# CodyRichter/MLMicroserviceTemplate

Measured on AMD Instinct MI355X. Metric: requests/sec (whole node) + p50 latency, ResNet-50 bs=32, higher is better.
Workload: dtype bf16; 1 GPU; model=resnet50-v1.5, global_batch=32, per_gpu_batch=32, image_size=224, parallelism=dp1, backend=fused, concurrent_slots=True, cu_partitions=2, hipgraph=True, inflight=4, numa_bound=True, partition_mode=intra, prestage=False, ranks_consistent=True, dist_backend=none, dist_world=1

## Files before the change

mlmicroservicetemplate_amd/ops/csrc/conv_chain.hip:

```cpp
#include "common.h"
#include "fastdiv.h"

namespace {

#define LDS3 __attribute__((address_space(3)))

MLS_DEV void glds16(rsrc_t r, char* lds, int voff, int soff) {
  __builtin_amdgcn_raw_ptr_buffer_load_lds(r, (LDS3 void*)lds, 16, voff, soff, 0, 0);
}

typedef unsigned int u32x4v __attribute__((__vector_size__(16)));

MLS_DEV uint32_t lds_off(const void* p);
MLS_DEV u32x4v lds_ld16_issue(uint32_t off);
template <typename T>
MLS_DEV void lds_landed(T& v);

#define CONST4 __attribute__((address_space(4)))

MLS_DEV f32x4 bias4(const float* b, int nt0, int fq) {
  if (!b) return f32x4{0.f, 0.f, 0.f, 0.f};
  const CONST4 f32x4* bp = (const CONST4 f32x4*)(b + nt0);
  const f32x4 b0 = bp[0], b1 = bp[1], b2 = bp[2], b3 = bp[3];
  return fq == 0 ? b0 : fq == 1 ? b1 : fq == 2 ? b2 : b3;
}

struct ChainArgs {
  const bf16* a1;
  const bf16* a2;
  const bf16* w3;
  const float* b3;
  const bf16* res;
  bf16* y;
  const bf16* w1;
  const float* b1;
  bf16* t1;
  int M, Ka, Kb, N1, N2;
  int Ho, Wo, H2, W2, stride2;
  FastDiv fd_howo, fd_wo;
  uint32_t a1_bytes, a2_bytes, w3_bytes, res_bytes, y_bytes, w1_bytes, t1_bytes;
  const bf16* t1in;
  const bf16* w2;
  const float* b2;
  uint32_t t1in_bytes, w2_bytes;
};

template <int CPR>
MLS_DEV int row_swz(int r) {
  if constexpr (CPR == 8) return r & 7;
  else return (r & 1) | ((r >> 1) & 2);
}

template <int BM, int KS, int N1, int N2, int CW, int OCC, bool SW, bool C2 = false>
__global__ __launch_bounds__(512, OCC) void conv_chain_kernel(const ChainArgs a) {
  constexpr int NW = 8, NT = 512, WM = 4, WN = 2;
  constexpr int WTM = BM / WM, TM = WTM / 16;
  constexpr int TN = CW / WN / 16;
  constexpr int TN2 = N2 / WN / 16;
  constexpr int CPR = CW / 8;
  constexpr int RPP = 64 / CPR;
  constexpr int A1_BYTES = BM * KS * 128;
  constexpr int W3_BYTES = CW * KS * 128;
  constexpr int W1_BYTES = N2 * CW * 2;
  constexpr int R_BYTES = BM * CW * 2;
  constexpr int STAGE = W3_BYTES + W1_BYTES + R_BYTES;
  constexpr int EPI_BYTES = BM * N2 * 2;
  constexpr int RING = A1_BYTES + 2 * STAGE;
  constexpr int LDS_BYTES = RING > EPI_BYTES ? RING : EPI_BYTES;
  constexpr int A1_PW = BM / 8 * KS / NW;
  constexpr int A1_S0 = C2 ? 1 : 0;
  constexpr int A1_PWL = BM / 8 * (KS - A1_S0) / NW;
  constexpr int W3_PW = CW / 8 * KS / NW;
  constexpr int W1_PW = N2 / RPP / NW;
  constexpr int R_PW = BM / RPP / NW;
  constexpr int Y_ST = BM * CPR / NT;
  constexpr int T_ST = BM * N2 / 8 / NT;
  constexpr int NJ = N1 / CW;
  static_assert(TM >= 1 && TN >= 1 && TN2 >= 1 && (CW == 64 || CW == 32), "tile");
  static_assert(A1_PW * NW * 8 == BM * KS && W3_PW * NW * 8 == CW * KS, "A1 / W3 DMA split");
  static_assert(W1_PW * NW * RPP == N2 && R_PW * NW * RPP == BM, "W1 / residual DMA split");
  static_assert(Y_ST * NT == BM * CPR && T_ST * NT == BM * N2 / 8, "epilogue split");
  static_assert(LDS_BYTES <= 160 * 1024, "LDS");
  __shared__ __attribute__((aligned(16))) char smem[LDS_BYTES];

  const int tid = threadIdx.x, lane = tid & 63;
  const int wid = __builtin_amdgcn_readfirstlane(tid >> 6);
  const int wm = wid / WN, wn = wid % WN;
  const int fr = lane & 15, fq = lane >> 4;
  const int m0 = xcd_remap(blockIdx.x, gridDim.x) * BM;
  const int K1 = a.Ka + a.Kb, KSA = a.Ka / 64;
  const bool has_res = a.res != nullptr;

  float b3v[SW ? 1 : NJ][TN], b1v[TN2];
  if constexpr (!SW) {
#pragma unroll
    for (int j = 0; j < NJ; ++j)
#pragma unroll
      for (int jn = 0; jn < TN; ++jn) b3v[j][jn] = a.b3 ? a.b3[j * CW + wn * (CW / 2) + jn * 16 + fr] : 0.f;
#pragma unroll
    for (int jn = 0; jn < TN2; ++jn) b1v[jn] = a.b1 ? a.b1[wn * (N2 / 2) + jn * 16 + fr] : 0.f;
  }

  const int r8 = lane >> 3, lc = (lane & 7) ^ r8;
  const int rq = lane / CPR, lq = (lane % CPR) ^ row_swz<CPR>(rq);

  const rsrc_t a1r = make_rsrc(a.a1, a.a1_bytes);
  const rsrc_t a2r = make_rsrc(a.a2, a.a2_bytes);
  const rsrc_t w3r = make_rsrc(a.w3, a.w3_bytes);
  const rsrc_t w1r = make_rsrc(a.w1, a.w1_bytes);
  const rsrc_t rr = make_rsrc(a.res, a.res_bytes);
  const rsrc_t yr = make_rsrc(a.y, a.y_bytes);
  const rsrc_t tr = make_rsrc(a.t1, a.t1_bytes);

  char* const sA1 = smem;
  auto stage_base = [&](int buf) { return smem + A1_BYTES + buf * STAGE; };

#pragma unroll
  for (int i = 0; i < A1_PWL; ++i) {
    const int q = A1_S0 * (BM / 8) + wid * A1_PWL + i;
    const int s = q / (BM / 8), rb = q - s * (BM / 8);
    const int m = m0 + rb * 8 + r8;
    char* dst = sA1 + q * 1024;
    if (s < KSA) {
      glds16(a1r, dst, m < a.M ? (m * a.Ka + s * 64 + lc * 8) * 2 : OOB, 0);
    } else {
      int off = OOB;
      if (m < a.M) {
        const int b = fastdiv(m, a.fd_howo), rem = m - b * (a.Ho * a.Wo);
        const int oh = fastdiv(rem, a.fd_wo), ow = rem - oh * a.Wo;
        off = (((b * a.H2 + oh * a.stride2) * a.W2 + ow * a.stride2) * a.Kb + (s - KSA) * 64 + lc * 8) * 2;
      }
      glds16(a2r, dst, off, 0);
    }
  }

  auto issue = [&](int j, int buf) {
    char* sW3 = stage_base(buf);
    char* sW1 = sW3 + W3_BYTES;
    char* sR = sW1 + W1_BYTES;
#pragma unroll
    for (int i = 0; i < W3_PW; ++i) {
      const int q = wid * W3_PW + i;
      const int s = q / (CW / 8), rb = q - s * (CW / 8);
      glds16(w3r, sW3 + q * 1024, ((j * CW + rb * 8 + r8) * K1 + s * 64 + lc * 8) * 2, 0);
    }
#pragma unroll
    for (int i = 0; i < W1_PW; ++i) {
      const int q = wid * W1_PW + i;
      glds16(w1r, sW1 + q * 1024, ((q * RPP + rq) * N1 + j * CW + lq * 8) * 2, 0);
    }
    if (has_res) {
#pragma unroll
      for (int i = 0; i < R_PW; ++i) {
        const int q = wid * R_PW + i;
        const int m = m0 + q * RPP + rq;
        glds16(rr, sR + q * 1024, m < a.M ? (m * N1 + j * CW + lq * 8) * 2 : OOB, 0);
      }
    }
  };

  if constexpr (C2) {
    constexpr int TAPS = 9, TSLOTS = 4, TAHEAD = 3, SROWS = 256, TNP = 64 / WN / 16;
    static_assert(BM == 128 && STAGE >= SROWS * 128 && STAGE >= TSLOTS * 8192, "strip / tap ring alias one stage each");
    char* const sS = stage_base(0);
    char* const sT = stage_base(1);
    const rsrc_t t1r = make_rsrc(a.t1in, a.t1in_bytes);
    const rsrc_t w2r = make_rsrc(a.w2, a.w2_bytes);
    const int halo = a.Wo + 1;
#pragma unroll
    for (int i = 0; i < SROWS / 8 / NW; ++i) {
      const int q = wid * (SROWS / 8 / NW) + i;
      const int sr = q * 8 + r8, p = m0 - halo + sr;
      glds16(t1r, sS + q * 1024, (p >= 0 && p < a.M && sr < BM + 2 * halo) ? (p * 64 + lc * 8) * 2 : OOB, 0);
    }
    auto issue_tap = [&](int t) {
      glds16(w2r, sT + (t % TSLOTS) * 8192 + wid * 1024, (((wid * 8 + r8) * TAPS + t) * 64 + lc * 8) * 2, 0);
    };
#pragma unroll
    for (int t = 0; t < TAHEAD; ++t) issue_tap(t);

    int okm[TM];
#pragma unroll
    for (int i = 0; i < TM; ++i) {
      const int m = m0 + wm * WTM + i * 16 + fr;
      okm[i] = 0;
      if (m < a.M) {
        const int b = fastdiv(m, a.fd_howo), rem = m - b * (a.Ho * a.Wo);
        const int oh = fastdiv(rem, a.fd_wo), ow = rem - oh * a.Wo;
#pragma unroll
        for (int t = 0; t < TAPS; ++t)
          if ((unsigned)(oh + t / 3 - 1) < (unsigned)a.Ho && (unsigned)(ow + t % 3 - 1) < (unsigned)a.Wo)
            okm[i] |= 1 << t;
      }
    }

    f32x4 accp[TM][TNP];
#pragma unroll
    for (int i = 0; i < TM; ++i)
#pragma unroll
      for (int jn = 0; jn < TNP; ++jn) accp[i][jn] = f32x4{0.f, 0.f, 0.f, 0.f};
#pragma unroll
    for (int t = 0; t < TAPS; ++t) {
      if (t + 2 < TAPS) asm volatile("s_waitcnt vmcnt(2)" ::: "memory");
      else if (t + 1 < TAPS) asm volatile("s_waitcnt vmcnt(1)" ::: "memory");
      else asm volatile("s_waitcnt vmcnt(0)" ::: "memory");
      asm volatile("s_waitcnt lgkmcnt(0)" ::: "memory");
      __builtin_amdgcn_s_barrier();
      if (t + TAHEAD < TAPS) issue_tap(t + TAHEAD);
      const int shift = halo + (t / 3 - 1) * a.Wo + (t % 3 - 1);
      const uint32_t oS = lds_off(sS), oT = lds_off(sT + (t % TSLOTS) * 8192);
      u32x4v av[2][TM], bv[2][TNP];
#pragma unroll
      for (int kk = 0; kk < 2; ++kk) {
        const int ch = fq + 4 * kk;
#pragma unroll
        for (int i = 0; i < TM; ++i) {
          const int r = wm * WTM + i * 16 + fr + shift;
          av[kk][i] = lds_ld16_issue(oS + (r * 8 + (ch ^ (r & 7))) * 16);
        }
#pragma unroll
        for (int jn = 0; jn < TNP; ++jn) {
          const int n = wn * 32 + jn * 16 + fr;
          bv[kk][jn] = lds_ld16_issue(oT + (n * 8 + (ch ^ (n & 7))) * 16);
        }
      }
#pragma unroll
      for (int kk = 0; kk < 2; ++kk) {
#pragma unroll
        for (int i = 0; i < TM; ++i) lds_landed(av[kk][i]);
#pragma unroll
        for (int jn = 0; jn < TNP; ++jn) lds_landed(bv[kk][jn]);
      }
#pragma unroll
      for (int kk = 0; kk < 2; ++kk) {
        bf16x8 af[TM], bfv[TNP];
#pragma unroll
        for (int i = 0; i < TM; ++i) {
          u32x4v v = av[kk][i];
          if (!((okm[i] >> t) & 1)) v = u32x4v{0u, 0u, 0u, 0u};
          af[i] = __builtin_bit_cast(bf16x8, v);
        }
#pragma unroll
        for (int jn = 0; jn < TNP; ++jn) bfv[jn] = __builtin_bit_cast(bf16x8, bv[kk][jn]);
#pragma unroll
        for (int i = 0; i < TM; ++i)
#pragma unroll
          for (int jn = 0; jn < TNP; ++jn)
            accp[i][jn] = __builtin_amdgcn_mfma_f32_16x16x32_bf16(bfv[jn], af[i], accp[i][jn], 0, 0, 0);
      }
    }
#pragma unroll
    for (int jn = 0; jn < TNP; ++jn) {
      const int nt0 = wn * 32 + jn * 16, col = nt0 + fq * 4;
      const f32x4 bb = bias4(a.b2, nt0, fq);
#pragma unroll
      for (int i = 0; i < TM; ++i) {
        const int row = wm * WTM + i * 16 + fr;
        bf16x4 q;
#pragma unroll
        for (int r = 0; r < 4; ++r) {
          const float e = accp[i][jn][r];
          q[r] = (bf16)fmaxf(e + bb[r], 0.f);
        }
        *reinterpret_cast<uint2*>(sA1 + row * 128 + (((col >> 3) ^ (row & 7)) << 4) + (col & 7) * 2) =
            __builtin_bit_cast(uint2, q);
      }
    }
    asm volatile("s_waitcnt lgkmcnt(0)" ::: "memory");
    __builtin_amdgcn_s_barrier();
  }
  issue(0, 0);

  f32x4 acc2[TM][TN2];
#pragma unroll
  for (int i = 0; i < TM; ++i)
#pragma unroll
    for (int jn = 0; jn < TN2; ++jn) acc2[i][jn] = f32x4{0.f, 0.f, 0.f, 0.f};

#pragma unroll
  for (int j = 0; j < NJ; ++j) {
    if (j == 0) {
      asm volatile("s_waitcnt vmcnt(0)" ::: "memory");
      if constexpr (!SW) {
#pragma unroll
        for (int jj = 0; jj < NJ; ++jj)
#pragma unroll
          for (int jn = 0; jn < TN; ++jn) asm volatile("" ::"v"(b3v[jj][jn]));
#pragma unroll
        for (int jn = 0; jn < TN2; ++jn) asm volatile("" ::"v"(b1v[jn]));
      }
    } else {
      asm volatile("s_waitcnt vmcnt(%0)" ::"n"(Y_ST) : "memory");
    }
    asm volatile("s_waitcnt lgkmcnt(0)" ::: "memory");
    __builtin_amdgcn_s_barrier();
    if (j + 1 < NJ) issue(j + 1, (j + 1) & 1);
    char* sW3 = stage_base(j & 1);
    char* sW1 = sW3 + W3_BYTES;
    char* sR = sW1 + W1_BYTES;

    f32x4 acc1[TM][TN];
#pragma unroll
    for (int i = 0; i < TM; ++i)
#pragma unroll
      for (int jn = 0; jn < TN; ++jn) acc1[i][jn] = f32x4{0.f, 0.f, 0.f, 0.f};
    const uint4* A1s = reinterpret_cast<const uint4*>(sA1);
    const uint4* W3s = reinterpret_cast<const uint4*>(sW3);
#pragma unroll
    for (int kk = 0; kk < 2 * KS; ++kk) {
      const int s = kk >> 1, ch = fq + 4 * (kk & 1);
      bf16x8 af[TM], bfv[TN];
#pragma unroll
      for (int i = 0; i < TM; ++i) {
        const int r = wm * WTM + i * 16 + fr;
        af[i] = __builtin_bit_cast(bf16x8, A1s[s * BM * 8 + r * 8 + (ch ^ (r & 7))]);
      }
#pragma unroll
      for (int jn = 0; jn < TN; ++jn) {
        const int n = wn * (CW / 2) + jn * 16 + fr;
        bfv[jn] = __builtin_bit_cast(bf16x8, W3s[s * CW * 8 + n * 8 + (ch ^ (n & 7))]);
      }
#pragma unroll
      for (int i = 0; i < TM; ++i)
#pragma unroll
        for (int jn = 0; jn < TN; ++jn)
          acc1[i][jn] = SW ? __builtin_amdgcn_mfma_f32_16x16x32_bf16(bfv[jn], af[i], acc1[i][jn], 0, 0, 0)
                                       : __builtin_amdgcn_mfma_f32_16x16x32_bf16(af[i], bfv[jn], acc1[i][jn], 0, 0, 0);
    }

    if constexpr (SW) {
#pragma unroll
      for (int jn = 0; jn < TN; ++jn) {
        const int nt0 = wn * (CW / 2) + jn * 16, col = nt0 + fq * 4;
        const f32x4 bb = bias4(a.b3, j * CW + nt0, fq);
#pragma unroll
        for (int i = 0; i < TM; ++i) {
          const int row = wm * WTM + i * 16 + fr;
          uint2* p = reinterpret_cast<uint2*>(sR + row * (CW * 2) + (((col >> 3) ^ row_swz<CPR>(row)) << 4) +
                                              (col & 7) * 2);
          float rs[4] = {0.f, 0.f, 0.f, 0.f};
          if (has_res) {
            const bf16x4 rv = __builtin_bit_cast(bf16x4, *p);
#pragma unroll
            for (int r = 0; r < 4; ++r) rs[r] = (float)rv[r];
          }
          bf16x4 q;
#pragma unroll
          for (int r = 0; r < 4; ++r) {
            const float e = acc1[i][jn][r];
            q[r] = (bf16)fmaxf(e + bb[r] + rs[r], 0.f);
          }
          *p = __builtin_bit_cast(uint2, q);
        }
      }
    } else
#pragma unroll
    for (int jn = 0; jn < TN; ++jn) {
      const int col = wn * (CW / 2) + jn * 16 + fr;
      const float bb = b3v[j][jn];
#pragma unroll
      for (int i = 0; i < TM; ++i)
#pragma unroll
        for (int r = 0; r < 4; ++r) {
          const int row = wm * WTM + i * 16 + fq * 4 + r;
          bf16* p = reinterpret_cast<bf16*>(sR + row * (CW * 2) + (((col >> 3) ^ row_swz<CPR>(row)) << 4) +
                                            (col & 7) * 2);
          const float e = acc1[i][jn][r];
          float v = e + bb;
          if (has_res) v += (float)*p;
          *p = (bf16)fmaxf(v, 0.f);
        }
    }
    asm volatile("s_waitcnt lgkmcnt(0)" ::: "memory");
    __builtin_amdgcn_s_barrier();

#pragma unroll
    for (int it = 0; it < Y_ST; ++it) {
      const int q = tid + it * NT;
      const int row = q / CPR, c = q % CPR;
      const uint4 v = *reinterpret_cast<const uint4*>(sR + row * (CW * 2) + ((c ^ row_swz<CPR>(row)) << 4));
      const int m = m0 + row;
      __builtin_amdgcn_raw_buffer_store_b128(__builtin_bit_cast(u32x4v, v), yr,
                                             m < a.M ? (m * N1 + j * CW + c * 8) * 2 : OOB, 0, 0);
    }

    const uint4* Ys = reinterpret_cast<const uint4*>(sR);
    const uint4* W1s = reinterpret_cast<const uint4*>(sW1);
#pragma unroll
    for (int kk = 0; kk < CW / 32; ++kk) {
      const int ch = fq + 4 * kk;
      bf16x8 af[TM], bfv[TN2];
#pragma unroll
      for (int i = 0; i < TM; ++i) {
        const int r = wm * WTM + i * 16 + fr;
        af[i] = __builtin_bit_cast(bf16x8, Ys[r * CPR + (ch ^ row_swz<CPR>(r))]);
      }
#pragma unroll
      for (int jn = 0; jn < TN2; ++jn) {
        const int n = wn * (N2 / 2) + jn * 16 + fr;
        bfv[jn] = __builtin_bit_cast(bf16x8, W1s[n * CPR + (ch ^ row_swz<CPR>(n))]);
      }
#pragma unroll
      for (int i = 0; i < TM; ++i)
#pragma unroll
        for (int jn = 0; jn < TN2; ++jn)
          acc2[i][jn] = SW ? __builtin_amdgcn_mfma_f32_16x16x32_bf16(bfv[jn], af[i], acc2[i][jn], 0, 0, 0)
                                       : __builtin_amdgcn_mfma_f32_16x16x32_bf16(af[i], bfv[jn], acc2[i][jn], 0, 0, 0);
    }
  }

  asm volatile("s_waitcnt lgkmcnt(0)" ::: "memory");
  __builtin_amdgcn_s_barrier();
  constexpr int TPR = N2 / 8;
  bf16* to = reinterpret_cast<bf16*>(smem);
  if constexpr (SW) {
#pragma unroll
    for (int jn = 0; jn < TN2; ++jn) {
      const int nt0 = wn * (N2 / 2) + jn * 16, col = nt0 + fq * 4;
      const f32x4 bb = bias4(a.b1, nt0, fq);
#pragma unroll
      for (int i = 0; i < TM; ++i) {
        const int row = wm * WTM + i * 16 + fr;
        bf16x4 q;
#pragma unroll
        for (int r = 0; r < 4; ++r) {
          const float e = acc2[i][jn][r];
          q[r] = (bf16)fmaxf(e + bb[r], 0.f);
        }
        *reinterpret_cast<uint2*>(to + row * N2 + ((((col >> 3) ^ (row & 7))) << 3) + (col & 7)) =
            __builtin_bit_cast(uint2, q);
      }
    }
  } else
#pragma unroll
  for (int jn = 0; jn < TN2; ++jn) {
    const int col = wn * (N2 / 2) + jn * 16 + fr;
    const float bb = b1v[jn];
#pragma unroll
    for (int i = 0; i < TM; ++i)
#pragma unroll
      for (int r = 0; r < 4; ++r) {
        const int row = wm * WTM + i * 16 + fq * 4 + r;
        const float e = acc2[i][jn][r];
        to[row * N2 + ((((col >> 3) ^ (row & 7))) << 3) + (col & 7)] = (bf16)fmaxf(e + bb, 0.f);
      }
  }
  asm volatile("s_waitcnt lgkmcnt(0)" ::: "memory");
  __builtin_amdgcn_s_barrier();
#pragma unroll
  for (int it = 0; it < T_ST; ++it) {
    const int q = tid + it * NT;
    const int row = q / TPR, c = q - (q / TPR) * TPR;
    const uint4 v = *reinterpret_cast<const uint4*>(to + row * N2 + ((c ^ (row & 7)) << 3));
    const int m = m0 + row;
    __builtin_amdgcn_raw_buffer_store_b128(__builtin_bit_cast(u32x4v, v), tr, m < a.M ? (m * a.N2 + c * 8) * 2 : OOB,
                                           0, 0);
  }
}

MLS_DEV void vm_wait(int n) {
#define MLS_VMW(k) \
  case k: asm volatile("s_waitcnt vmcnt(" #k ")" ::: "memory"); break;
  switch (n) {
    MLS_VMW(1) MLS_VMW(2) MLS_VMW(3) MLS_VMW(4) MLS_VMW(5) MLS_VMW(6) MLS_VMW(7) MLS_VMW(8) MLS_VMW(9) MLS_VMW(10)
    MLS_VMW(11) MLS_VMW(12) MLS_VMW(13) MLS_VMW(14) MLS_VMW(15) MLS_VMW(16) MLS_VMW(17) MLS_VMW(18) MLS_VMW(19)
    MLS_VMW(20)
    default: asm volatile("s_waitcnt vmcnt(0)" ::: "memory");
  }
#undef MLS_VMW
}

MLS_DEV uint32_t lds_off(const void* p) { return (uint32_t)(uintptr_t)(LDS3 const char*)p; }
MLS_DEV uint2 lds_ld8_issue(uint32_t off) {
  uint2 v;
  asm volatile("ds_read_b64 %0, %1" : "=v"(v) : "v"(off) : "memory");
  return v;
}
MLS_DEV uint32_t lds_ld2_issue(uint32_t off) {
  uint32_t v;
  asm volatile("ds_read_u16 %0, %1" : "=v"(v) : "v"(off) : "memory");
  return v;
}
template <typename T>
MLS_DEV void lds_landed(T& v) { asm volatile("s_waitcnt lgkmcnt(0)" : "+v"(v)::"memory"); }
MLS_DEV u32x4v lds_ld16_issue(uint32_t off) {
  u32x4v v;
  asm volatile("ds_read_b128 %0, %1" : "=v"(v) : "v"(off) : "memory");
  return v;
}
MLS_DEV uint4 lds_ld16(uint32_t off) {
  uint4 v;
  asm volatile("ds_read_b128 %0, %1\n\ts_waitcnt lgkmcnt(0)" : "=v"(v) : "v"(off) : "memory");
  return v;
}
MLS_DEV void lds_st8(uint32_t off, uint2 v) { asm volatile("ds_write_b64 %0, %1" ::"v"(off), "v"(v) : "memory"); }
MLS_DEV void lds_st2(uint32_t off, bf16 h) {
  const uint32_t v = __builtin_bit_cast(unsigned short, h);
  asm volatile("ds_write_b16 %0, %1" ::"v"(off), "v"(v) : "memory");
}

template <int BM, int KS, int N1, int N2, int CW, int S, int OCC, bool SW, bool PERS>
__global__ __launch_bounds__(512, OCC) void conv_chain_ring_kernel(const ChainArgs a, const int ntiles) {
  constexpr int NW = 8, NT = 512, WM = 4, WN = 2;
  constexpr int WTM = BM / WM, TM = WTM / 16;
  constexpr int TN = CW / WN / 16;
  constexpr int TN2 = N2 / WN / 16;
  constexpr int CPR = CW / 8;
  constexpr int RPP = 64 / CPR;
  constexpr int NJ = N1 / CW;
  constexpr int A1_BYTES = BM * KS * 128;
  constexpr int W3_BYTES = CW * KS * 128;
  constexpr int W1_BYTES = N2 * CW * 2;
  constexpr int R_BYTES = BM * CW * 2;
  constexpr int EPI_BYTES = BM * N2 * 2;
  constexpr int STAGE = PERS ? R_BYTES : W3_BYTES + W1_BYTES + R_BYTES;
  constexpr int OFF_W3 = (PERS ? 2 : 1) * A1_BYTES;
  constexpr int OFF_W1 = OFF_W3 + (PERS ? NJ * W3_BYTES : 0);
  constexpr int OFF_EPI = OFF_W1 + (PERS ? NJ * W1_BYTES : 0);
  constexpr int OFF_RING = OFF_EPI + (PERS ? EPI_BYTES : 0);
  constexpr int RING_END = OFF_RING + S * STAGE;
  constexpr int LDS_BYTES = RING_END > EPI_BYTES ? RING_END : EPI_BYTES;
  constexpr int A1_P = BM / 8 * KS, W3_P = CW / 8 * KS, W1_P = N2 / RPP, R_P = BM / RPP;
  constexpr int Y_ST = BM * CPR / NT;
  constexpr int T_ST = BM * N2 / 8 / NT;
  static_assert(TM >= 1 && TN >= 1 && TN2 >= 1 && (CW == 64 || CW == 32), "tile");
  static_assert(S >= 2 && S - 1 <= NJ && (!PERS || NJ % S == 0), "ring depth");
  static_assert(Y_ST * NT == BM * CPR && T_ST * NT == BM * N2 / 8, "epilogue split");
  static_assert(LDS_BYTES <= 160 * 1024, "LDS");
  __shared__ __attribute__((aligned(16))) char smem[LDS_BYTES];

  const int tid = threadIdx.x, lane = tid & 63;
  const int wid = __builtin_amdgcn_readfirstlane(tid >> 6);
  const int wm = wid / WN, wn = wid % WN;
  const int fr = lane & 15, fq = lane >> 4;
  const int G = gridDim.x;
  int tile = chain_first_tile(blockIdx.x, G);
  if (tile >= ntiles) return;
  int m0 = tile * BM;
  const int K1 = a.Ka + a.Kb, KSA = a.Ka / 64;
  const bool has_res = a.res != nullptr;

  float b3v[SW ? 1 : NJ][TN], b1v[TN2];
  if constexpr (!SW) {
#pragma unroll
    for (int j = 0; j < NJ; ++j)
#pragma unroll
      for (int jn = 0; jn < TN; ++jn) b3v[j][jn] = a.b3 ? a.b3[j * CW + wn * (CW / 2) + jn * 16 + fr] : 0.f;
#pragma unroll
    for (int jn = 0; jn < TN2; ++jn) b1v[jn] = a.b1 ? a.b1[wn * (N2 / 2) + jn * 16 + fr] : 0.f;
  }

  const int r8 = lane >> 3, lc = (lane & 7) ^ r8;
  const int rq = lane / CPR, lq = (lane % CPR) ^ row_swz<CPR>(rq);

  const rsrc_t a1r = make_rsrc(a.a1, a.a1_bytes);
  const rsrc_t a2r = make_rsrc(a.a2, a.a2_bytes);
  const rsrc_t w3r = make_rsrc(a.w3, a.w3_bytes);
  const rsrc_t w1r = make_rsrc(a.w1, a.w1_bytes);
  const rsrc_t rr = make_rsrc(a.res, a.res_bytes);
  const rsrc_t yr = make_rsrc(a.y, a.y_bytes);
  const rsrc_t tr = make_rsrc(a.t1, a.t1_bytes);

  auto pieces = [&](int P) { return P / NW + (wid < P % NW ? 1 : 0); };
  const int n_a1 = pieces(A1_P);
  const int n_st = (PERS ? 0 : pieces(W3_P) + pieces(W1_P)) + (has_res ? pieces(R_P) : 0);

  auto issue_a1 = [&](int mt, char* dstA) {
#pragma unroll
    for (int i = 0; i < (A1_P + NW - 1) / NW; ++i) {
      const int q = i * NW + wid;
      if (A1_P % NW != 0 && q >= A1_P) break;
      const int s = q / (BM / 8), rb = q - s * (BM / 8);
      const int m = mt + rb * 8 + r8;
      char* dst = dstA + q * 1024;
      if (s < KSA) {
        glds16(a1r, dst, m < a.M ? (m * a.Ka + s * 64 + lc * 8) * 2 : OOB, 0);
      } else {
        int off = OOB;
        if (m < a.M) {
          const int b = fastdiv(m, a.fd_howo), rem = m - b * (a.Ho * a.Wo);
          const int oh = fastdiv(rem, a.fd_wo), ow = rem - oh * a.Wo;
          off = (((b * a.H2 + oh * a.stride2) * a.W2 + ow * a.stride2) * a.Kb + (s - KSA) * 64 + lc * 8) * 2;
        }
        glds16(a2r, dst, off, 0);
      }
    }
  };
  auto issue_w = [&](int j, char* sW3, char* sW1) {
#pragma unroll
    for (int i = 0; i < (W3_P + NW - 1) / NW; ++i) {
      const int q = i * NW + wid;
      if (W3_P % NW != 0 && q >= W3_P) break;
      const int s = q / (CW / 8), rb = q - s * (CW / 8);
      glds16(w3r, sW3 + q * 1024, ((j * CW + rb * 8 + r8) * K1 + s * 64 + lc * 8) * 2, 0);
    }
#pragma unroll
    for (int i = 0; i < (W1_P + NW - 1) / NW; ++i) {
      const int q = i * NW + wid;
      if (W1_P % NW != 0 && q >= W1_P) break;
      glds16(w1r, sW1 + q * 1024, ((q * RPP + rq) * N1 + j * CW + lq * 8) * 2, 0);
    }
  };
  auto issue_r = [&](int j, int mt, char* sR) {
    if (!has_res) return;
#pragma unroll
    for (int i = 0; i < (R_P + NW - 1) / NW; ++i) {
      const int q = i * NW + wid;
      if (R_P % NW != 0 && q >= R_P) break;
      const int m = mt + q * RPP + rq;
      glds16(rr, sR + q * 1024, m < a.M ? (m * N1 + j * CW + lq * 8) * 2 : OOB, 0);
    }
  };
  auto w3_at = [&](int j, int slot) { return smem + (PERS ? OFF_W3 + j * W3_BYTES : OFF_RING + slot * STAGE); };
  auto w1_at = [&](int j, int slot) {
    return smem + (PERS ? OFF_W1 + j * W1_BYTES : OFF_RING + slot * STAGE + W3_BYTES);
  };
  auto r_at = [&](int slot) { return smem + OFF_RING + slot * STAGE + (PERS ? 0 : W3_BYTES + W1_BYTES); };
  auto issue_stage = [&](int j, int slot, int mt) {
    if constexpr (!PERS) issue_w(j, w3_at(j, slot), w1_at(j, slot));
    issue_r(j, mt, r_at(slot));
  };

  if constexpr (PERS) {
#pragma unroll
    for (int j = 0; j < NJ; ++j) issue_w(j, w3_at(j, 0), w1_at(j, 0));
  }
  issue_a1(m0, smem);
#pragma unroll
  for (int s = 0; s < S - 1; ++s) issue_stage(s, s, m0);
  if constexpr (PERS) {
    asm volatile("s_waitcnt vmcnt(0)" ::: "memory");
    if constexpr (!SW) {
#pragma unroll
      for (int jj = 0; jj < NJ; ++jj)
#pragma unroll
        for (int jn = 0; jn < TN; ++jn) asm volatile("" ::"v"(b3v[jj][jn]));
#pragma unroll
      for (int jn = 0; jn < TN2; ++jn) asm volatile("" ::"v"(b1v[jn]));
    }
  }

  f32x4 acc2[TM][TN2];
#pragma unroll
  for (int i = 0; i < TM; ++i)
#pragma unroll
    for (int jn = 0; jn < TN2; ++jn) acc2[i][jn] = f32x4{0.f, 0.f, 0.f, 0.f};

  int abuf = 0;
  bool first = true;
  for (;;) {
    int m0n = a.M;
    if constexpr (PERS) {
      const int next = chain_next_tile(tile, G);
      if (next < ntiles) m0n = next * BM;
    }
    char* const sA1 = smem + abuf * A1_BYTES;

#pragma unroll
    for (int j = 0; j < NJ; ++j) {
      if constexpr (PERS) {
        const int jm = j < S - 1 ? j : S - 1;
        const int ahead = (S - 2) * n_st + (j >= NJ - S + 2 ? n_a1 : 0);
        vm_wait(ahead + (first ? jm * Y_ST : (S - 1) * Y_ST + (j <= S - 2 ? T_ST : 0)));
      } else {
        const int left = NJ - 1 - j < S - 2 ? NJ - 1 - j : S - 2;
        const int jm = j < S - 1 ? j : S - 1;
        vm_wait(left * n_st + jm * Y_ST);
        if (!SW && j == 0) {
#pragma unroll
          for (int jj = 0; jj < NJ; ++jj)
#pragma unroll
            for (int jn = 0; jn < TN; ++jn) asm volatile("" ::"v"(b3v[jj][jn]));
#pragma unroll
          for (int jn = 0; jn < TN2; ++jn) asm volatile("" ::"v"(b1v[jn]));
        }
      }
      asm volatile("s_waitcnt lgkmcnt(0)" ::: "memory");
      __builtin_amdgcn_s_barrier();
      {
        const int jn = j + S - 1;
        if (jn < NJ) {
          issue_stage(jn, jn % S, m0);
        } else if (PERS) {
          if (jn == NJ) issue_a1(m0n, smem + (abuf ^ 1) * A1_BYTES);
          issue_stage(jn - NJ, jn % S, m0n);
        }
      }
      char* const sW3 = w3_at(j, j % S);
      char* const sW1 = w1_at(j, j % S);
      char* const sR = r_at(j % S);

      f32x4 acc1[TM][TN];
#pragma unroll
      for (int i = 0; i < TM; ++i)
#pragma unroll
        for (int jn = 0; jn < TN; ++jn) acc1[i][jn] = f32x4{0.f, 0.f, 0.f, 0.f};
      const uint4* A1s = reinterpret_cast<const uint4*>(sA1);
      const uint4* W3s = reinterpret_cast<const uint4*>(sW3);
#pragma unroll
      for (int kk = 0; kk < 2 * KS; ++kk) {
        const int s = kk >> 1, ch = fq + 4 * (kk & 1);
        bf16x8 af[TM], bfv[TN];
#pragma unroll
        for (int i = 0; i < TM; ++i) {
          const int r = wm * WTM + i * 16 + fr;
          af[i] = __builtin_bit_cast(bf16x8, A1s[s * BM * 8 + r * 8 + (ch ^ (r & 7))]);
        }
#pragma unroll
        for (int jn = 0; jn < TN; ++jn) {
          const int n = wn * (CW / 2) + jn * 16 + fr;
          bfv[jn] = __builtin_bit_cast(bf16x8, W3s[s * CW * 8 + n * 8 + (ch ^ (n & 7))]);
        }
#pragma unroll
        for (int i = 0; i < TM; ++i)
#pragma unroll
          for (int jn = 0; jn < TN; ++jn)
            acc1[i][jn] = SW ? __builtin_amdgcn_mfma_f32_16x16x32_bf16(bfv[jn], af[i], acc1[i][jn], 0, 0, 0)
                             : __builtin_amdgcn_mfma_f32_16x16x32_bf16(af[i], bfv[jn], acc1[i][jn], 0, 0, 0);
      }

      auto y_at = [&](int row, int col) {
        return lds_off(sR + row * (CW * 2) + (((col >> 3) ^ row_swz<CPR>(row)) << 4) + (col & 7) * 2);
      };
      if constexpr (SW) {
        uint2 rv[TN][TM];
        if (has_res) {
#pragma unroll
          for (int jn = 0; jn < TN; ++jn)
#pragma unroll
            for (int i = 0; i < TM; ++i)
              rv[jn][i] = lds_ld8_issue(y_at(wm * WTM + i * 16 + fr, wn * (CW / 2) + jn * 16 + fq * 4));
#pragma unroll
          for (int jn = 0; jn < TN; ++jn)
#pragma unroll
            for (int i = 0; i < TM; ++i) lds_landed(rv[jn][i]);
        }
#pragma unroll
        for (int jn = 0; jn < TN; ++jn) {
          const int nt0 = wn * (CW / 2) + jn * 16, col = nt0 + fq * 4;
          const f32x4 bb = bias4(a.b3, j * CW + nt0, fq);
#pragma unroll
          for (int i = 0; i < TM; ++i) {
            const int row = wm * WTM + i * 16 + fr;
            float rs[4] = {0.f, 0.f, 0.f, 0.f};
            if (has_res) {
              const bf16x4 r4 = __builtin_bit_cast(bf16x4, rv[jn][i]);
#pragma unroll
              for (int r = 0; r < 4; ++r) rs[r] = (float)r4[r];
            }
            bf16x4 q;
#pragma unroll
            for (int r = 0; r < 4; ++r) {
              const float e = acc1[i][jn][r];
              q[r] = (bf16)fmaxf(e + bb[r] + rs[r], 0.f);
            }
            lds_st8(y_at(row, col), __builtin_bit_cast(uint2, q));
          }
        }
      } else {
        uint32_t rv[TN][TM][4];
        if (has_res) {
#pragma unroll
          for (int jn = 0; jn < TN; ++jn)
#pragma unroll
            for (int i = 0; i < TM; ++i)
#pragma unroll
              for (int r = 0; r < 4; ++r)
                rv[jn][i][r] = lds_ld2_issue(y_at(wm * WTM + i * 16 + fq * 4 + r, wn * (CW / 2) + jn * 16 + fr));
#pragma unroll
          for (int jn = 0; jn < TN; ++jn)
#pragma unroll
            for (int i = 0; i < TM; ++i)
#pragma unroll
              for (int r = 0; r < 4; ++r) lds_landed(rv[jn][i][r]);
        }
#pragma unroll
        for (int jn = 0; jn < TN; ++jn) {
          const int col = wn * (CW / 2) + jn * 16 + fr;
          const float bb = b3v[j][jn];
#pragma unroll
          for (int i = 0; i < TM; ++i)
#pragma unroll
            for (int r = 0; r < 4; ++r) {
              const int row = wm * WTM + i * 16 + fq * 4 + r;
              const float e = acc1[i][jn][r];
              float v = e + bb;
              if (has_res) v += (float)__builtin_bit_cast(bf16, (unsigned short)rv[jn][i][r]);
              lds_st2(y_at(row, col), (bf16)fmaxf(v, 0.f));
            }
        }
      }
      asm volatile("s_waitcnt lgkmcnt(0)" ::: "memory");
      __builtin_amdgcn_s_barrier();

#pragma unroll
      for (int it = 0; it < Y_ST; ++it) {
        const int q = tid + it * NT;
        const int row = q / CPR, c = q % CPR;
        const uint4 v = lds_ld16(lds_off(sR + row * (CW * 2) + ((c ^ row_swz<CPR>(row)) << 4)));
        const int m = m0 + row;
        __builtin_amdgcn_raw_buffer_store_b128(__builtin_bit_cast(u32x4v, v), yr,
                                               m < a.M ? (m * N1 + j * CW + c * 8) * 2 : OOB, 0, 0);
      }

      const uint4* Ys = reinterpret_cast<const uint4*>(sR);
      const uint4* W1s = reinterpret_cast<const uint4*>(sW1);
#pragma unroll
      for (int kk = 0; kk < CW / 32; ++kk) {
        const int ch = fq + 4 * kk;
        bf16x8 af[TM], bfv[TN2];
#pragma unroll
        for (int i = 0; i < TM; ++i) {
          const int r = wm * WTM + i * 16 + fr;
          af[i] = __builtin_bit_cast(bf16x8, Ys[r * CPR + (ch ^ row_swz<CPR>(r))]);
        }
#pragma unroll
        for (int jn = 0; jn < TN2; ++jn) {
          const int n = wn * (N2 / 2) + jn * 16 + fr;
          bfv[jn] = __builtin_bit_cast(bf16x8, W1s[n * CPR + (ch ^ row_swz<CPR>(n))]);
        }
#pragma unroll
        for (int i = 0; i < TM; ++i)
#pragma unroll
          for (int jn = 0; jn < TN2; ++jn)
            acc2[i][jn] = SW ? __builtin_amdgcn_mfma_f32_16x16x32_bf16(bfv[jn], af[i], acc2[i][jn], 0, 0, 0)
                             : __builtin_amdgcn_mfma_f32_16x16x32_bf16(af[i], bfv[jn], acc2[i][jn], 0, 0, 0);
      }
    }

    constexpr int TPR = N2 / 8;
    bf16* to = reinterpret_cast<bf16*>(smem + (PERS ? OFF_EPI : 0));
    if constexpr (!PERS) {
      asm volatile("s_waitcnt lgkmcnt(0)" ::: "memory");
      __builtin_amdgcn_s_barrier();
    }
    if constexpr (SW) {
#pragma unroll
      for (int jn = 0; jn < TN2; ++jn) {
        const int nt0 = wn * (N2 / 2) + jn * 16, col = nt0 + fq * 4;
        const f32x4 bb = bias4(a.b1, nt0, fq);
#pragma unroll
        for (int i = 0; i < TM; ++i) {
          const int row = wm * WTM + i * 16 + fr;
          bf16x4 q;
#pragma unroll
          for (int r = 0; r < 4; ++r) {
            const float e = acc2[i][jn][r];
            q[r] = (bf16)fmaxf(e + bb[r], 0.f);
          }
          lds_st8(lds_off(to + row * N2 + ((((col >> 3) ^ (row & 7))) << 3) + (col & 7)), __builtin_bit_cast(uint2, q));
        }
      }
    } else {
#pragma unroll
      for (int jn = 0; jn < TN2; ++jn) {
        const int col = wn * (N2 / 2) + jn * 16 + fr;
        const float bb = b1v[jn];
#pragma unroll
        for (int i = 0; i < TM; ++i)
#pragma unroll
          for (int r = 0; r < 4; ++r) {
            const int row = wm * WTM + i * 16 + fq * 4 + r;
            const float e = acc2[i][jn][r];
            lds_st2(lds_off(to + row * N2 + ((((col >> 3) ^ (row & 7))) << 3) + (col & 7)), (bf16)fmaxf(e + bb, 0.f));
          }
      }
    }
    asm volatile("s_waitcnt lgkmcnt(0)" ::: "memory");
    __builtin_amdgcn_s_barrier();
#pragma unroll
    for (int it = 0; it < T_ST; ++it) {
      const int q = tid + it * NT;
      const int row = q / TPR, c = q - (q / TPR) * TPR;
      const uint4 v = lds_ld16(lds_off(to + row * N2 + ((c ^ (row & 7)) << 3)));
      const int m = m0 + row;
      __builtin_amdgcn_raw_buffer_store_b128(__builtin_bit_cast(u32x4v, v), tr,
                                             m < a.M ? (m * a.N2 + c * 8) * 2 : OOB, 0, 0);
    }
    if constexpr (!PERS) break;
    tile = chain_next_tile(tile, G);
    if (tile >= ntiles) break;
    m0 = m0n;
    abuf ^= 1;
    first = false;
#pragma unroll
    for (int i = 0; i < TM; ++i)
#pragma unroll
      for (int jn = 0; jn < TN2; ++jn) acc2[i][jn] = f32x4{0.f, 0.f, 0.f, 0.f};
  }
  if constexpr (PERS) asm volatile("s_waitcnt vmcnt(0)" ::: "memory");
}

template <int KS, int N1, int N2, int CW, int BM = 128, bool C2 = false>
int launch_chain(const ChainArgs& a, hipStream_t st) {
  constexpr int LDS = BM * KS * 128 + 2 * (CW * KS * 128 + N2 * CW * 2 + BM * CW * 2);
  constexpr int OCC = LDS <= 80 * 1024 ? 4 : 2;
#ifdef MLS_CHAIN_SWAP
  constexpr bool SW = MLS_CHAIN_SWAP;
#else
  constexpr bool SW = KS == 1;
#endif
  hipLaunchKernelGGL((conv_chain_kernel<BM, KS, N1, N2, CW, OCC, SW, C2>), dim3((unsigned)((a.M + BM - 1) / BM)),
                     dim3(512), 0, st, a);
  return (int)hipGetLastError();
}

int g_chain_grid = 0;

template <int BM, int KS, int N1, int N2, int CW, int S, bool PERS>
int launch_ring(const ChainArgs& a, hipStream_t st) {
#ifdef MLS_CHAIN_SWAP
  constexpr bool SW = MLS_CHAIN_SWAP;
#else
  constexpr bool SW = KS == 1;
#endif
  constexpr int LDS = PERS ? 2 * BM * KS * 128 + N1 * KS * 128 + N2 * N1 * 2 + BM * N2 * 2 + S * BM * CW * 2
                            : BM * KS * 128 + S * (CW * KS * 128 + N2 * CW * 2 + BM * CW * 2);
  constexpr int OCC = LDS <= 80 * 1024 ? 4 : 2;
  const int ntiles = (a.M + BM - 1) / BM;
  int grid = ntiles;
  if (PERS) {
    const int cus = mls_num_cus();
    grid = g_chain_grid > 0 ? g_chain_grid : (ntiles < cus ? ntiles : cus);
  }
  hipLaunchKernelGGL((conv_chain_ring_kernel<BM, KS, N1, N2, CW, S, OCC, SW, PERS>), dim3((unsigned)grid), dim3(512), 0,
                     st, a, ntiles);
  return (int)hipGetLastError();
}

int g_chain_cw_l2 = 0;
int g_chain_bm_l2 = 128;
int g_chain_variant = 0;

constexpr bool RING_L1_DUAL = false, RING_L2 = true, RING_L2_OUT = false;

bool use_ring(bool shape_default) { return g_chain_variant == 2 || (g_chain_variant == 0 && shape_default); }

}

extern "C" {

int mls_conv_chain(const void* a1, const void* a2, const void* w3, const float* b3, const void* res, void* y,
                   const void* w1, const float* b1, void* t1, int B, int Ho, int Wo, int Ka, int H2, int W2, int Kb,
                   int stride2, int N1, int N2, void* stream) {
  if (B <= 0 || Ho <= 0 || Wo <= 0 || Ka <= 0 || Ka % 64 || Kb < 0 || Kb % 64 || N1 <= 0 || N1 % 64 || N2 <= 0)
    return MLS_BAD_ARG;
  if (Kb > 0 && (stride2 < 1 || (Ho - 1) * stride2 >= H2 || (Wo - 1) * stride2 >= W2 || res)) return MLS_BAD_ARG;
  ChainArgs a{};
  a.a1 = (const bf16*)a1;
  a.a2 = (const bf16*)a2;
  a.w3 = (const bf16*)w3;
  a.b3 = b3;
  a.res = (const bf16*)res;
  a.y = (bf16*)y;
  a.w1 = (const bf16*)w1;
  a.b1 = b1;
  a.t1 = (bf16*)t1;
  a.M = B * Ho * Wo;
  a.Ka = Ka;
  a.Kb = Kb;
  a.N1 = N1;
  a.N2 = N2;
  a.Ho = Ho, a.Wo = Wo, a.H2 = H2, a.W2 = W2, a.stride2 = stride2;
  a.fd_howo = fastdiv_make((uint32_t)(Ho * Wo));
  a.fd_wo = fastdiv_make((uint32_t)Wo);
  const long M = a.M;
  const long sizes[7] = {M * Ka * 2, (long)B * H2 * W2 * Kb * 2, (long)N1 * (Ka + Kb) * 2, res ? M * N1 * 2 : 0,
                         M * N1 * 2, (long)N2 * N1 * 2, M * N2 * 2};
  for (long s : sizes)
    if (s >= 0x7fffffffL) return MLS_UNSUPPORTED;
  a.a1_bytes = (uint32_t)sizes[0];
  a.a2_bytes = (uint32_t)sizes[1];
  a.w3_bytes = (uint32_t)sizes[2];
  a.res_bytes = (uint32_t)sizes[3];
  a.y_bytes = (uint32_t)sizes[4];
  a.w1_bytes = (uint32_t)sizes[5];
  a.t1_bytes = (uint32_t)sizes[6];
  const hipStream_t st = (hipStream_t)stream;
  const int ks = (Ka + Kb) / 64;
  if (ks == 1 && N1 == 256 && N2 == 64) return launch_chain<1, 256, 64, 64>(a, st);
  if (ks == 2 && N1 == 256 && N2 == 64)
    return use_ring(RING_L1_DUAL) ? launch_ring<64, 2, 256, 64, 64, 2, true>(a, st)
                                  : launch_chain<2, 256, 64, 64>(a, st);
  if (ks == 1 && N1 == 256 && N2 == 128) return launch_chain<1, 256, 128, 64>(a, st);
  const bool l2_override = g_chain_variant == 0 && (g_chain_bm_l2 == 64 || g_chain_cw_l2 != 0);
  if (ks == 2 && N1 == 512 && N2 == 128) {
    if (!l2_override && use_ring(RING_L2)) return launch_ring<128, 2, 512, 128, 64, 2, false>(a, st);
    if (g_chain_bm_l2 == 64) return launch_chain<2, 512, 128, 64, 64>(a, st);
    return g_chain_cw_l2 == 32 ? launch_chain<2, 512, 128, 32>(a, st) : launch_chain<2, 512, 128, 64>(a, st);
  }
  if (ks == 2 && N1 == 512 && N2 == 256) {
    if (!l2_override && use_ring(RING_L2_OUT)) return launch_ring<128, 2, 512, 256, 32, 3, false>(a, st);
    return g_chain_bm_l2 == 64 ? launch_chain<2, 512, 256, 64, 64>(a, st) : launch_chain<2, 512, 256, 32>(a, st);
  }
  if (ks == 4 && N1 == 1024 && N2 == 256) return launch_chain<4, 1024, 256, 32>(a, st);
  return MLS_UNSUPPORTED;
}

int mls_conv_chain_conv2(const void* t1_in, const void* w2, const float* b2, const void* a2, const void* w3,
                         const float* b3, const void* res, void* y, const void* w1, const float* b1, void* t1, int B,
                         int H, int W, int Ka, int H2, int W2, int Kb, int stride2, int N1, int N2, void* stream) {
  if (B <= 0 || H <= 0 || W <= 0 || Ka <= 0 || Kb < 0 || Kb % 64 || N1 <= 0 || N1 % 64 || N2 <= 0) return MLS_BAD_ARG;
  if (Kb > 0 && (stride2 < 1 || (H - 1) * stride2 >= H2 || (W - 1) * stride2 >= W2 || res)) return MLS_BAD_ARG;
  if (Ka != 64 || 2 * (W + 1) + 128 > 256) return MLS_UNSUPPORTED;
  ChainArgs a{};
  a.t1in = (const bf16*)t1_in;
  a.w2 = (const bf16*)w2;
  a.b2 = b2;
  a.a2 = (const bf16*)a2;
  a.w3 = (const bf16*)w3;
  a.b3 = b3;
  a.res = (const bf16*)res;
  a.y = (bf16*)y;
  a.w1 = (const bf16*)w1;
  a.b1 = b1;
  a.t1 = (bf16*)t1;
  a.Ka = Ka;
  a.Kb = Kb;
  a.N1 = N1;
  a.N2 = N2;
  a.Ho = H, a.Wo = W, a.H2 = H2, a.W2 = W2, a.stride2 = stride2;
  a.fd_howo = fastdiv_make((uint32_t)(H * W));
  a.fd_wo = fastdiv_make((uint32_t)W);
  const long M = (long)B * H * W;
  const long sizes[7] = {M * Ka * 2, (long)B * H2 * W2 * Kb * 2, (long)N1 * (Ka + Kb) * 2, res ? M * N1 * 2 : 0,
                         M * N1 * 2, (long)N2 * N1 * 2, M * N2 * 2};
  for (long s : sizes)
    if (s >= 0x7fffffffL) return MLS_UNSUPPORTED;
  a.M = (int)M;
  a.t1in_bytes = (uint32_t)sizes[0];
  a.a2_bytes = (uint32_t)sizes[1];
  a.w3_bytes = (uint32_t)sizes[2];
  a.res_bytes = (uint32_t)sizes[3];
  a.y_bytes = (uint32_t)sizes[4];
  a.w1_bytes = (uint32_t)sizes[5];
  a.t1_bytes = (uint32_t)sizes[6];
  a.w2_bytes = 64 * 9 * 64 * 2;
  const hipStream_t st = (hipStream_t)stream;
  const int ks = (Ka + Kb) / 64;
  if (ks == 1 && N1 == 256 && N2 == 64) return launch_chain<1, 256, 64, 64, 128, true>(a, st);
  if (ks == 2 && N1 == 256 && N2 == 64) return launch_chain<2, 256, 64, 64, 128, true>(a, st);
  if (ks == 1 && N1 == 256 && N2 == 128) return launch_chain<1, 256, 128, 64, 128, true>(a, st);
  return MLS_UNSUPPORTED;
}

void mls_chain_set_l2_cw(int cw) { g_chain_cw_l2 = (cw == 32 || cw == 64) ? cw : 0; }

void mls_chain_set_l2_bm(int bm) { g_chain_bm_l2 = bm == 64 ? 64 : 128; }


void mls_chain_set_variant(int v) { g_chain_variant = (v == 1 || v == 2) ? v : 0; }

void mls_chain_set_grid(int g) { g_chain_grid = g > 0 ? g : 0; }

}

MLS_DEBUG_EXPORT(conv_chain)
```

Measured before the change: 58660 requests/s.

## Route layer3 chain through ring kernel with A1 tile held in registers

Adds an AREG variant of the non-persistent ring kernel. The A1 activation tile is staged once through the last ring slot, loaded into per-wave registers, and its dedicated LDS region is dropped, so the next stage's prefetch is issued only after the first GEMM has consumed the borrowed slot. The ks=4, N1=1024, N2=256 (layer3) chain now uses this ring path with BM=64, CW=64 and S=2 instead of the plain chain kernel. The aim is a smaller LDS footprint and pipelined weight/residual loads for that shape. The cost is extra register pressure and a later prefetch issue, which reduces the overlap.

Result: no change. 58600 requests/s (-0.1%).

```diff
diff --git a/mlmicroservicetemplate_amd/ops/csrc/conv_chain.hip b/mlmicroservicetemplate_amd/ops/csrc/conv_chain.hip
--- a/mlmicroservicetemplate_amd/ops/csrc/conv_chain.hip
+++ b/mlmicroservicetemplate_amd/ops/csrc/conv_chain.hip
@@ -499,7 +499,7 @@
   asm volatile("ds_write_b16 %0, %1" ::"v"(off), "v"(v) : "memory");
 }
 
-template <int BM, int KS, int N1, int N2, int CW, int S, int OCC, bool SW, bool PERS>
+template <int BM, int KS, int N1, int N2, int CW, int S, int OCC, bool SW, bool PERS, bool AREG = false>
 __global__ __launch_bounds__(512, OCC) void conv_chain_ring_kernel(const ChainArgs a, const int ntiles) {
   constexpr int NW = 8, NT = 512, WM = 4, WN = 2;
   constexpr int WTM = BM / WM, TM = WTM / 16;
@@ -514,7 +514,7 @@
   constexpr int R_BYTES = BM * CW * 2;
   constexpr int EPI_BYTES = BM * N2 * 2;
   constexpr int STAGE = PERS ? R_BYTES : W3_BYTES + W1_BYTES + R_BYTES;
-  constexpr int OFF_W3 = (PERS ? 2 : 1) * A1_BYTES;
+  constexpr int OFF_W3 = (PERS ? 2 : AREG ? 0 : 1) * A1_BYTES;
   constexpr int OFF_W1 = OFF_W3 + (PERS ? NJ * W3_BYTES : 0);
   constexpr int OFF_EPI = OFF_W1 + (PERS ? NJ * W1_BYTES : 0);
   constexpr int OFF_RING = OFF_EPI + (PERS ? EPI_BYTES : 0);
@@ -526,6 +526,7 @@
   static_assert(TM >= 1 && TN >= 1 && TN2 >= 1 && (CW == 64 || CW == 32), "tile");
   static_assert(S >= 2 && S - 1 <= NJ && (!PERS || NJ % S == 0), "ring depth");
   static_assert(Y_ST * NT == BM * CPR && T_ST * NT == BM * N2 / 8, "epilogue split");
+  static_assert(!AREG || (!PERS && A1_BYTES <= STAGE), "the A1 image borrows the last ring slot for one tile");
   static_assert(LDS_BYTES <= 160 * 1024, "LDS");
   __shared__ __attribute__((aligned(16))) char smem[LDS_BYTES];
 
@@ -625,9 +626,27 @@
 #pragma unroll
     for (int j = 0; j < NJ; ++j) issue_w(j, w3_at(j, 0), w1_at(j, 0));
   }
-  issue_a1(m0, smem);
+  char* const a1_img = smem + (AREG ? OFF_RING + (S - 1) * STAGE : 0);
+  issue_a1(m0, a1_img);
 #pragma unroll
   for (int s = 0; s < S - 1; ++s) issue_stage(s, s, m0);
+  u32x4v a1f[AREG ? 2 * KS : 1][TM];
+  if constexpr (AREG) {
+    asm volatile("s_waitcnt vmcnt(0)" ::: "memory");
+    __builtin_amdgcn_s_barrier();
+    const uint32_t oA = lds_off(a1_img);
+#pragma unroll
+    for (int kk = 0; kk < 2 * KS; ++kk)
+#pragma unroll
+      for (int i = 0; i < TM; ++i) {
+        const int r = wm * WTM + i * 16 + fr, ch = fq + 4 * (kk & 1);
+        a1f[kk][i] = lds_ld16_issue(oA + ((kk >> 1) * BM * 8 + r * 8 + (ch ^ (r & 7))) * 16);
+      }
+#pragma unroll
+    for (int kk = 0; kk < 2 * KS; ++kk)
+#pragma unroll
+      for (int i = 0; i < TM; ++i) lds_landed(a1f[kk][i]);
+  }
   if constexpr (PERS) {
     asm volatile("s_waitcnt vmcnt(0)" ::: "memory");
     if constexpr (!SW) {
@@ -654,7 +673,7 @@
       const int next = chain_next_tile(tile, G);
       if (next < ntiles) m0n = next * BM;
     }
-    char* const sA1 = smem + abuf * A1_BYTES;
+    char* const sA1 = AREG ? a1_img : smem + abuf * A1_BYTES;
 
 #pragma unroll
     for (int j = 0; j < NJ; ++j) {
@@ -677,7 +696,7 @@
       }
       asm volatile("s_waitcnt lgkmcnt(0)" ::: "memory");
       __builtin_amdgcn_s_barrier();
-      {
+      auto issue_next = [&]() {
         const int jn = j + S - 1;
         if (jn < NJ) {
           issue_stage(jn, jn % S, m0);
@@ -685,7 +704,8 @@
           if (jn == NJ) issue_a1(m0n, smem + (abuf ^ 1) * A1_BYTES);
           issue_stage(jn - NJ, jn % S, m0n);
         }
-      }
+      };
+      if constexpr (!AREG) issue_next();
       char* const sW3 = w3_at(j, j % S);
       char* const sW1 = w1_at(j, j % S);
       char* const sR = r_at(j % S);
@@ -704,7 +724,8 @@
 #pragma unroll
         for (int i = 0; i < TM; ++i) {
           const int r = wm * WTM + i * 16 + fr;
-          af[i] = __builtin_bit_cast(bf16x8, A1s[s * BM * 8 + r * 8 + (ch ^ (r & 7))]);
+          if constexpr (AREG) af[i] = __builtin_bit_cast(bf16x8, a1f[kk][i]);
+          else af[i] = __builtin_bit_cast(bf16x8, A1s[s * BM * 8 + r * 8 + (ch ^ (r & 7))]);
         }
 #pragma unroll
         for (int jn = 0; jn < TN; ++jn) {
@@ -718,6 +739,7 @@
             acc1[i][jn] = SW ? __builtin_amdgcn_mfma_f32_16x16x32_bf16(bfv[jn], af[i], acc1[i][jn], 0, 0, 0)
                              : __builtin_amdgcn_mfma_f32_16x16x32_bf16(af[i], bfv[jn], acc1[i][jn], 0, 0, 0);
       }
+      if constexpr (AREG) issue_next();
 
       auto y_at = [&](int row, int col) {
         return lds_off(sR + row * (CW * 2) + (((col >> 3) ^ row_swz<CPR>(row)) << 4) + (col & 7) * 2);
@@ -907,7 +929,7 @@
 
 int g_chain_grid = 0;
 
-template <int BM, int KS, int N1, int N2, int CW, int S, bool PERS>
+template <int BM, int KS, int N1, int N2, int CW, int S, bool PERS, bool AREG = false>
 int launch_ring(const ChainArgs& a, hipStream_t st) {
 #ifdef MLS_CHAIN_SWAP
   constexpr bool SW = MLS_CHAIN_SWAP;
@@ -915,7 +937,7 @@
   constexpr bool SW = KS == 1;
 #endif
   constexpr int LDS = PERS ? 2 * BM * KS * 128 + N1 * KS * 128 + N2 * N1 * 2 + BM * N2 * 2 + S * BM * CW * 2
-                            : BM * KS * 128 + S * (CW * KS * 128 + N2 * CW * 2 + BM * CW * 2);
+                            : (AREG ? 0 : BM * KS * 128) + S * (CW * KS * 128 + N2 * CW * 2 + BM * CW * 2);
   constexpr int OCC = LDS <= 80 * 1024 ? 4 : 2;
   const int ntiles = (a.M + BM - 1) / BM;
   int grid = ntiles;
@@ -923,7 +945,7 @@
     const int cus = mls_num_cus();
     grid = g_chain_grid > 0 ? g_chain_grid : (ntiles < cus ? ntiles : cus);
   }
-  hipLaunchKernelGGL((conv_chain_ring_kernel<BM, KS, N1, N2, CW, S, OCC, SW, PERS>), dim3((unsigned)grid), dim3(512), 0,
+  hipLaunchKernelGGL((conv_chain_ring_kernel<BM, KS, N1, N2, CW, S, OCC, SW, PERS, AREG>), dim3((unsigned)grid), dim3(512), 0,
                      st, a, ntiles);
   return (int)hipGetLastError();
 }
@@ -932,7 +954,7 @@
 int g_chain_bm_l2 = 128;
 int g_chain_variant = 0;
 
-constexpr bool RING_L1_DUAL = false, RING_L2 = true, RING_L2_OUT = false;
+constexpr bool RING_L1_DUAL = false, RING_L2 = true, RING_L2_OUT = false, RING_L3 = true;
 
 bool use_ring(bool shape_default) { return g_chain_variant == 2 || (g_chain_variant == 0 && shape_default); }
 
@@ -993,7 +1015,9 @@
     if (!l2_override && use_ring(RING_L2_OUT)) return launch_ring<128, 2, 512, 256, 32, 3, false>(a, st);
     return g_chain_bm_l2 == 64 ? launch_chain<2, 512, 256, 64, 64>(a, st) : launch_chain<2, 512, 256, 32>(a, st);
   }
-  if (ks == 4 && N1 == 1024 && N2 == 256) return launch_chain<4, 1024, 256, 32>(a, st);
+  if (ks == 4 && N1 == 1024 && N2 == 256)
+    return use_ring(RING_L3) ? launch_ring<64, 4, 1024, 256, 64, 2, false, true>(a, st)
+                             : launch_chain<4, 1024, 256, 32>(a, st);
   return MLS_UNSUPPORTED;
 }
 
```
